# nanoporetech/pomfret

Measured on AMD Instinct MI355X. Metric: aligned reads/sec (methphase kernel), higher is better.
Workload: dtype u32/f32

## Files before the change

### include/pomfret_amd.h

```cpp
#ifndef POMFRET_AMD_H
#define POMFRET_AMD_H

#include <stddef.h>
#include <stdint.h>

#ifdef __cplusplus
extern "C" {
#endif

#define PF_ABI_VERSION 1

#define PF_OK               0
#define PF_ERR_ARG         -1
#define PF_ERR_HIP         -2
#define PF_ERR_NOMEM       -3
#define PF_ERR_UNSUPPORTED -4
#define PF_ERR_LIMIT       -5
#define PF_ERR_INTERNAL    -6

typedef struct pf_cfg {
    int32_t k;
    int32_t k_span;
    int32_t cov_for_selection;
    int32_t cov_for_runtime;
// ... 90 lines not shown
    const uint32_t *end;
    const uint64_t *cigar_off;
    const uint32_t *cigar;
    const uint64_t *seq_off;
    const uint32_t *seq_len;
    const uint8_t  *seq;
    const uint64_t *md_off;
    const char     *md;
} pf_read_aln_batch_t;


typedef struct pf_ctx pf_ctx_t;
typedef struct pf_dbatch pf_dbatch_t;

int  pf_abi_version(void);
int  pf_device_count(void);
const char *pf_strerror(int code);

int  pf_ctx_create(int device, pf_ctx_t **out);
void pf_ctx_destroy(pf_ctx_t *ctx);

int  pf_batch_upload(pf_ctx_t *ctx, const pf_cfg_t *cfg,
                     const pf_window_batch_t *batch, pf_dbatch_t **out);
void pf_batch_free(pf_dbatch_t *db);
uint32_t pf_batch_n_windows(const pf_dbatch_t *db);
uint32_t pf_batch_n_reads(const pf_dbatch_t *db);
uint64_t pf_batch_n_calls(const pf_dbatch_t *db);

int  pf_methphase_run(pf_ctx_t *ctx, pf_dbatch_t *db, pf_window_out_t *out);

int  pf_methphase_launch(pf_ctx_t *ctx, pf_dbatch_t *db);
int  pf_methphase_finish(pf_ctx_t *ctx, pf_dbatch_t *db, pf_window_out_t *out);

int  pf_batch_upload_aln(pf_ctx_t *ctx, const pf_cfg_t *cfg, const pf_load_cfg_t *lcfg,
                         const pf_aln_batch_t *aln, pf_dbatch_t **out);
int  pf_batch_read_recs(const pf_dbatch_t *db, uint32_t *rec_of_read, uint32_t n);
int64_t pf_batch_debug_calls(pf_dbatch_t *db, uint64_t *call_off, uint32_t *pos, uint8_t *cat,
                             uint32_t *first, uint32_t *last, uint64_t cap);

int  pf_batch_debug_recs(pf_dbatch_t *db, uint64_t *sizes, uint16_t *flag, uint8_t *mapq, uint32_t *pos,
                         uint32_t *l_qseq, float *de, uint8_t *hp, uint64_t *cigar_off, uint32_t *cigar,
                         uint64_t *seq_off, uint8_t *seq, uint64_t *mm_off, uint8_t *mm, uint64_t *ml_off,
                         uint8_t *ml);
int  pf_batch_load_counters(pf_dbatch_t *db, uint64_t *out, int n);

int  pf_methphase_windows(int device, const pf_cfg_t *cfg,
                          const pf_window_batch_t *batch, pf_window_out_t *out);

int  pf_last_kernel_times(pf_ctx_t *ctx, const char **names, float *ms, int *n);

int  pf_batch_stats(pf_dbatch_t *db, uint64_t *out, uint64_t n);
int  pf_batch_k3_paths(pf_dbatch_t *db, uint8_t *out, uint64_t n);
int  pf_batch_k12_paths(pf_dbatch_t *db, uint8_t *out, uint64_t n);

int  pf_batch_set_mask(pf_dbatch_t *db, const uint32_t *pos, uint64_t n, const uint32_t *win_rng);
int  pf_batch_masked_sites(pf_dbatch_t *db, uint32_t *out, uint64_t n);
int  pf_batch_k3_budget(const pf_dbatch_t *db, uint32_t *out, uint64_t n);

int  pf_batch_heavy(const pf_dbatch_t *db, uint32_t *probs, uint32_t cap);

int  pf_batch_debug_sites(pf_dbatch_t *db, uint32_t w, int dir, uint32_t *real,
                          uint32_t *starts, uint8_t *lens, uint32_t cap);
int64_t pf_batch_debug_methmers(pf_dbatch_t *db, int dir, uint32_t *mmr_n,
                                uint32_t *mmr_start, uint32_t *keys, uint64_t cap);

typedef struct pf_pileup {
    uint32_t n_windows;
    uint64_t n_sites;
    const uint64_t *win_off;
    const uint32_t *pos;
    const uint32_t *cnt;
    float ms_kernels;
} pf_pileup_t;
int  pf_batch_pileup(pf_ctx_t *ctx, pf_dbatch_t *db, const uint8_t *read_hp, uint32_t n_hp, pf_pileup_t **out);
void pf_pileup_free(pf_pileup_t *p);

typedef struct pf_dmr_cfg {
    uint32_t min_cov;
    uint32_t min_delta_pct;
    uint32_t max_gap;
    uint32_t min_sites;
} pf_dmr_cfg_t;

#define PF_DMR_OPEN_LEFT  1u
#define PF_DMR_OPEN_RIGHT 2u
typedef struct pf_dmr_run {
    uint32_t start;
    uint32_t end;
    uint32_t n_sites;
    int32_t  sign;
    uint64_t sum[4];
    uint32_t open;
    uint32_t reserved;
} pf_dmr_run_t;

typedef struct pf_dmr {
    uint64_t n_runs;
    const pf_dmr_run_t *runs;
    uint64_t n_informative;
    float ms_kernels;
    float ms_upload;
} pf_dmr_t;

int  pf_dmr_regions(pf_ctx_t *ctx, const pf_pileup_t *pile, uint32_t w0, uint32_t w1, const pf_dmr_cfg_t *cfg,
                    const uint32_t *breaks, uint32_t n_breaks, pf_dmr_t **out);
int  pf_dmr_regions_block(pf_ctx_t *ctx, const pf_pileup_t *pile, uint32_t w0, uint32_t w1, const pf_dmr_cfg_t *cfg,
// ... 490 lines not shown
```

### pomfret_amd/_lib.py

```python
from __future__ import annotations

import ctypes as C
import os
import weakref

import numpy as np

from .abi import (DMR_RUN_DTYPE, AlnBatch, AssignConfig, PfAssign, PfAssignCfg, Config, DmrConfig, KnownVars, LoadConfig, PfAlnBatch, PfCfg, PfDmr, PfDmrCfg,
                  PfKnownVars, PfLoadCfg, PfPerm, PfPileup, PfReadAlnBatch, PfTagcheck, PfWindowBatch, PfWindowOut, ReadAlnBatch,
                  WindowBatch, WindowResult)

_HERE = os.path.dirname(os.path.abspath(__file__))
LIB_PATH = os.path.join(_HERE, "libpomfret_amd.so")
_lib = None


class PomfretError(RuntimeError):
    pass


def lib():
    global _lib
    if _lib is None:
        if not os.path.exists(LIB_PATH):
# ... 547 lines not shown
    def assign(self, cfg: AssignConfig = None, read_hp=None) -> dict:
        hp_ptr, n_hp = None, 0
        if read_hp is not None:
            hp = np.zeros(np.size(read_hp) + 1, np.uint8)
            hp[:-1] = np.asarray(read_hp, np.uint8).ravel()
            hp_ptr, n_hp = hp.ctypes.data, hp.size - 1
        c = (cfg or AssignConfig()).to_c()
        p = C.POINTER(PfAssign)()
        _check(lib().pf_batch_assign(self.ctx.handle, self.handle, hp_ptr, n_hp, C.byref(c), C.byref(p)), "pf_batch_assign")
        try:
            r = p.contents
            W, R = int(r.n_windows), int(r.n_reads)

            def arr(ptr, n, dt):
                return np.ctypeslib.as_array(ptr, (n,)).copy() if n else np.zeros(0, dt)
            return dict(win_read_off=arr(r.win_read_off, W + 1, np.uint32), n_used=arr(r.n_used, R, np.uint32),
                        llr=arr(r.llr, R, np.int64), hp=arr(r.hp, R, np.uint8),
                        win_n=arr(r.win_n, 3 * W, np.uint32).reshape(W, 3), ms=float(r.ms_kernels))
        finally:
            lib().pf_assign_free(p)

    def tagcheck(self, cfg: AssignConfig = None, read_hp=None) -> dict:
        hp_ptr, n_hp = None, 0
        if read_hp is not None:
            hp = np.zeros(np.size(read_hp) + 1, np.uint8)
            hp[:-1] = np.asarray(read_hp, np.uint8).ravel()
            hp_ptr, n_hp = hp.ctypes.data, hp.size - 1
        c = (cfg or AssignConfig()).to_c()
        p = C.POINTER(PfTagcheck)()
        _check(lib().pf_batch_tagcheck(self.ctx.handle, self.handle, hp_ptr, n_hp, C.byref(c), C.byref(p)),
               "pf_batch_tagcheck")
        try:
            r = p.contents
            W, R = int(r.n_windows), int(r.n_reads)

            def arr(ptr, n, dt):
                return np.ctypeslib.as_array(ptr, (n,)).copy() if n else np.zeros(0, dt)
            return dict(win_read_off=arr(r.win_read_off, W + 1, np.uint32), n_used=arr(r.n_used, R, np.uint32),
                        llr=arr(r.llr, R, np.int64), verdict=arr(r.verdict, R, np.uint8), hp=arr(r.hp, R, np.uint8),
                        win_n=arr(r.win_n, 8 * W, np.uint32).reshape(W, 2, 4), ms=float(r.ms_kernels))
        finally:
            lib().pf_tagcheck_free(p)

    def stats(self) -> np.ndarray:
        out = np.zeros((max(self.n_windows, 1), 2, 8), np.uint64)
        _check(lib().pf_batch_stats(self.handle, out.ctypes.data, out.size), "pf_batch_stats")
        return out[:self.n_windows]

    def k12_paths(self) -> np.ndarray:
        out = np.zeros(max(self.n_windows, 1), np.uint8)
        _check(lib().pf_batch_k12_paths(self.handle, out.ctypes.data, out.size), "pf_batch_k12_paths")
        return out[:self.n_windows]

    def set_mask(self, pos, win_rng=None):
        pos = np.ascontiguousarray(np.asarray(pos, np.int64).ravel())
        if pos.size and (pos.min() < 0 or pos.max() > 0xFFFFFFFF):
            raise PomfretError("pf_batch_set_mask: positions must fit 32 bits")
        p32 = np.ascontiguousarray(pos.astype(np.uint32))
        rng = None
        if win_rng is not None:
            rng = np.ascontiguousarray(np.asarray(win_rng, np.uint32).reshape(-1))
            if rng.size != 2 * self.n_windows:
                raise PomfretError(f"pf_batch_set_mask: win_rng needs {self.n_windows} (begin, end) pairs")
        _check(lib().pf_batch_set_mask(self.handle, p32.ctypes.data if p32.size else None, p32.size,
                                       rng.ctypes.data if rng is not None and rng.size else None),
               "pf_batch_set_mask")

    def masked_sites(self) -> np.ndarray:
        out = np.zeros(max(self.n_windows, 1), np.uint32)
        _check(lib().pf_batch_masked_sites(self.handle, out.ctypes.data, out.size), "pf_batch_masked_sites")
        return out[:self.n_windows]

    def k3_paths(self) -> np.ndarray:
        out = np.zeros(max(2 * self.n_windows, 2), np.uint8)
        _check(lib().pf_batch_k3_paths(self.handle, out.ctypes.data, out.size), "pf_batch_k3_paths")
        return out[:2 * self.n_windows].reshape(-1, 2)

    def k3_budget(self) -> dict:
        out = np.zeros(4, np.uint32)
        _check(lib().pf_batch_k3_budget(self.handle, out.ctypes.data, out.size), "pf_batch_k3_budget")
        return {"lds": int(out[0]), "resident": int(out[1]), "lds_heavy": int(out[2]), "n_heavy": int(out[3])}

    def heavy_problems(self) -> np.ndarray:
        n = lib().pf_batch_heavy(self.handle, None, 0)
        out = np.zeros(max(n, 1), np.uint32)
        if n:
            lib().pf_batch_heavy(self.handle, out.ctypes.data, n)
        return out[:n]

    def debug_sites(self, w: int, direction: int, cap: int = 1 << 22):
        real = np.zeros(cap, np.uint32)
        starts = np.zeros(cap, np.uint32)
        lens = np.zeros(cap, np.uint8)
        n = lib().pf_batch_debug_sites(self.handle, w, direction, real.ctypes.data,
                                       starts.ctypes.data, lens.ctypes.data, cap)
        if n < 0:
            _check(n, "pf_batch_debug_sites")
        return real[:n], starts[:n], lens[:n]

    def debug_methmers(self, direction: int, cap: int = 1 << 26):
        n = np.zeros(max(self.n_reads, 1), np.uint32)
        st = np.zeros(max(self.n_reads, 1), np.uint32)
        keys = np.zeros(cap, np.uint32)
        tot = lib().pf_batch_debug_methmers(self.handle, direction, n.ctypes.data, st.ctypes.data,
                                            keys.ctypes.data, cap)
        if tot < 0:
# ... 33 lines not shown
```

### pomfret_amd/csrc/pf_api.hip

```cpp
#include <hip/hip_runtime.h>
#include <mutex>
#include <stdint.h>
#include <stdio.h>
#include <stdlib.h>
#include <string.h>
#include <algorithm>
#include <thread>
#include <vector>
#include "pf_device.h"
#include "pf_load.h"
#include "pf_host.h"
#include "../../include/pomfret_amd.h"

__global__ void pf_k12_sites_methmers(pf_dev_batch d);
__global__ void pf_k2_methmers(pf_dev_batch d);
__global__ void pf_k12_chunks(pf_dev_batch d);
__global__ void pf_k3_greedy(pf_dev_batch d);
__global__ void pf_k3_wave(pf_dev_batch d);
__global__ void pf_k3_fallback(pf_dev_batch d);
__global__ void pf_k3_heavy(pf_dev_batch d);
__global__ void pf_k3_kdict(pf_dev_batch d);
__global__ void pf_k0_load(pf_load_dev d);
__global__ void pf_k0_multi(pf_load_dev d);
__global__ void pf_k0_scan(pf_load_dev d);
// ... 1500 lines not shown
}

extern "C" int64_t pf_batch_debug_methmers(pf_dbatch_t *b, int dir, uint32_t *mmr_n, uint32_t *mmr_start,
                                           uint32_t *keys, uint64_t cap) {
    if (!b || dir < 0 || dir > 1) return PF_ERR_ARG;
    const int rc = run_debug(b, 2);
    if (rc) return rc;
    std::vector<uint32_t> n(2ull * b->R), s0(2ull * b->R);
    std::vector<uint64_t> off(2ull * b->R);
    if (b->R) {
        HIPCHK(hipMemcpy(n.data(), b->d.mmr_n, 8ull * b->R, hipMemcpyDeviceToHost));
        HIPCHK(hipMemcpy(s0.data(), b->d.mmr_start, 8ull * b->R, hipMemcpyDeviceToHost));
        HIPCHK(hipMemcpy(off.data(), b->d.mmr_off, 16ull * b->R, hipMemcpyDeviceToHost));
    }
    uint64_t tot = 0;
    for (uint32_t r = 0; r < b->R; r++) {
        const uint64_t g = 2ull * r + dir;
        mmr_n[r] = n[g];
        mmr_start[r] = s0[g];
        if (tot + n[g] > cap) return PF_ERR_ARG;
        if (n[g]) HIPCHK(hipMemcpy(keys + tot, b->d.keys + off[g], 4ull * n[g], hipMemcpyDeviceToHost));
        tot += n[g];
    }
    return (int64_t)tot;
}

extern "C" int pf_batch_stats(pf_dbatch_t *b, uint64_t *out, uint64_t n) {
    if (!b || !out || n < 16ull * b->W) return PF_ERR_ARG;
    HIPCHK(hipSetDevice(b->ctx->device));
    HIPCHK(hipStreamSynchronize(b->ctx->stream));
    if (b->W) HIPCHK(hipMemcpy(out, b->d.stats, 16ull * b->W * sizeof(uint64_t), hipMemcpyDeviceToHost));
    for (uint64_t i = 0; i < 2ull * b->W; i++) out[i * 8 + 2] &= (1ull << 56) - 1;
    return PF_OK;
}

extern "C" int pf_batch_k3_paths(pf_dbatch_t *b, uint8_t *out, uint64_t n) {
    if (!b || !out || n < 2ull * b->W) return PF_ERR_ARG;
    HIPCHK(hipSetDevice(b->ctx->device));
    HIPCHK(hipStreamSynchronize(b->ctx->stream));
    std::vector<uint64_t> st(16ull * b->W + 1);
    if (b->W) HIPCHK(hipMemcpy(st.data(), b->d.stats, 16ull * b->W * sizeof(uint64_t), hipMemcpyDeviceToHost));
    for (uint64_t i = 0; i < 2ull * b->W; i++) out[i] = (uint8_t)(st[i * 8 + 2] >> 56);
    return PF_OK;
}

extern "C" int pf_batch_k12_paths(pf_dbatch_t *b, uint8_t *out, uint64_t n) {
    if (!b || !out || n < b->W) return PF_ERR_ARG;
    HIPCHK(hipSetDevice(b->ctx->device));
    HIPCHK(hipStreamSynchronize(b->ctx->stream));
    if (b->W) HIPCHK(hipMemcpy(out, b->d.k12_path, b->W, hipMemcpyDeviceToHost));
    return PF_OK;
}

extern "C" int pf_batch_k3_budget(const pf_dbatch_t *b, uint32_t *out, uint64_t n) {
    if (!b || !out || n < 4) return PF_ERR_ARG;
    HIPCHK(hipSetDevice(b->ctx->device));
    out[0] = b->d.lds_bytes;
    out[1] = k3_resident(b->ctx, b->d.lds_bytes);
    out[2] = b->d.lds_heavy;
    out[3] = b->n_heavy;
    return PF_OK;
}

extern "C" int pf_batch_heavy(const pf_dbatch_t *b, uint32_t *probs, uint32_t cap) {
    if (!b) return PF_ERR_ARG;
    for (uint32_t i = 0; i < b->n_heavy && i < cap && probs; i++) probs[i] = b->h_heavy[i];
    return (int)b->n_heavy;
}

extern "C" int pf_batch_prof(pf_dbatch_t *b, uint64_t *out, uint64_t n) {
    if (!b || !out || n < 80ull * b->W) return PF_ERR_ARG;
    HIPCHK(hipSetDevice(b->ctx->device));
    HIPCHK(hipStreamSynchronize(b->ctx->stream));
    if (b->W) HIPCHK(hipMemcpy(out, b->d.prof, 80ull * b->W * sizeof(uint64_t), hipMemcpyDeviceToHost));
    return PF_OK;
}

extern "C" void pf_ctx_set_haptag_ms(pf_ctx *c, float ms, const char *name) {
    c->haptag_ms = ms; c->have_haptag = 1; c->haptag_name = name;
}

extern "C" int pf_last_kernel_times(pf_ctx_t *ctx, const char **names, float *ms, int *n) {
    if (!ctx || !n) return PF_ERR_ARG;
    const int hv = ctx->heavy_ms >= 0.0f ? 1 : 0;
    const int tot = PF_NKERN + hv + (ctx->have_haptag ? 1 : 0);
    int m = *n < tot ? *n : tot;
    for (int i = 0; i < m; i++) {
        if (i < PF_NKERN) {
            if (names) names[i] = (i == 5 && ctx->k3_block) ? "pf_k3_greedy" : k_names[i];
            if (ms) ms[i] = ctx->have_times ? ctx->last_ms[i] : -1.0f;
        } else if (i == PF_NKERN && hv) {
            if (names) names[i] = "pf_k3_heavy";
            if (ms) ms[i] = ctx->heavy_ms;
        } else {
            if (names) names[i] = ctx->haptag_name;
            if (ms) ms[i] = ctx->haptag_ms;
        }
    }
    *n = tot;
    return PF_OK;
}

extern "C" int64_t pf_batch_debug_calls(pf_dbatch_t *b, uint64_t *call_off, uint32_t *pos, uint8_t *cat,
                                        uint32_t *first, uint32_t *last, uint64_t cap) {
    if (!b || !call_off || !pos || !cat || !first || !last) return PF_ERR_ARG;
    const int rc = run_debug(b, 0);
// ... 142 lines not shown
```

### pomfret_amd/csrc/pf_kernels.hip

```cpp
#include <hip/hip_runtime.h>
#include <stdint.h>
#include "pf_device.h"

#define DEV static __device__ __forceinline__

#ifdef PF_K3_PROFILE
DEV unsigned long long k3_stamp_now() {
    unsigned long long t;
    __builtin_amdgcn_sched_barrier(0);
    asm volatile("s_memtime %0\n\ts_waitcnt lgkmcnt(0)" : "=s"(t) :: "memory");
    __builtin_amdgcn_sched_barrier(0);
    return t;
}
#define K3_STAMP(i) do { const unsigned long long t_ = k3_stamp_now(); \
    prof_acc[i] += t_ - prof_last; prof_last = t_; } while (0)
DEV unsigned long long k3_realtime() {
    unsigned long long t;
    asm volatile("s_memrealtime %0\n\ts_waitcnt lgkmcnt(0)" : "=s"(t) :: "memory");
    return t;
}
#define K3_COUNT(i, v) do { prof_acc[i] += (v); } while (0)
#define K12_STAMP(i) do { if (threadIdx.x == 0) { const unsigned long long t_ = k3_stamp_now(); \
    d.prof[64ull * d.W + (uint64_t)w * 16 + (i)] = t_ - k12_t0; k12_t0 = t_; } } while (0)
#define K2_STAMP(i) do { if (k2acc) { const unsigned long long t_ = k3_stamp_now(); \
// ... 207 lines not shown
    for (uint64_t cb = c0 + lane; cb < c1; cb += 256) {
        uint32_t pos[4], prv[4], cat[4];
#pragma unroll
        for (int u = 0; u < 4; u++) {
            const uint64_t c = cb + 64 * u;
            const bool ok = c < c1;
            pos[u] = ok ? d.call_pos[c] : 0xFFFFFFFFu;
            prv[u] = (ok && c > c0) ? d.call_pos[c - 1] : 0xFFFFFFFFu;
            cat[u] = ok ? d.call_cat[c] : 2u;
        }
#pragma unroll
        for (int u = 0; u < 4; u++) {
            const uint64_t c = cb + 64 * u;
            const uint32_t p = pos[u];
            if (c < c1 && (c == c0 || prv[u] != p) && p >= plo && p <= phi) {
                uint32_t lo = qlo, hi = qhi;
                while (lo < hi) {
                    const uint32_t mid = (lo + hi) >> 1;
                    if (sp[mid] < p) lo = mid + 1; else hi = mid;
                }
                if (lo < qhi && sp[lo] == p) chars[lo - qlo] = (uint8_t)cat[u];
            }
        }
    }
    wave_sync();
}

DEV void wave_lb2(const uint32_t *a, uint32_t n, uint32_t kA, uint32_t kB, uint32_t lane, uint32_t &lbA,
                  uint32_t &lbB) {
    const uint32_t h = lane >> 5, j = lane & 31;
    const uint32_t key = h ? kB : kA;
    uint32_t lo = 0, hi = n;
    for (;;) {
        const uint32_t len = hi - lo;
        const uint32_t step = (len + 31) >> 5;
        const uint32_t p = lo + j * step;
        const bool lt = len > 0 && p < hi && a[p] < key;
        const uint64_t bal = __ballot(lt);
        const uint32_t c = (uint32_t)__popc((uint32_t)(bal >> (32 * h)));
        if (len > 0) {
            if (c == 0) hi = lo;
            else {
                const uint32_t pn = lo + c * step;
                lo = lo + (c - 1) * step + 1;
                hi = pn < hi ? pn : hi;
            }
        }
        if (__ballot(hi > lo) == 0) break;
    }
    lbA = rdl(lo, 0);
    lbB = rdl(lo, 32);
}

struct K2SiteHash {
    const uint32_t *t;
    uint32_t mask, pmin;
};
DEV uint32_t k2_hash_slot(uint32_t rel) { return (rel * 2654435761u) >> 7; }
DEV uint32_t k2_site_of(const K2SiteHash &hs, uint32_t p) {
    const uint32_t rel = p - hs.pmin;
    if (p < hs.pmin || rel >= (1u << 19)) return PF_NONE;
    uint32_t h = k2_hash_slot(rel) & hs.mask;
    for (;;) {
        const uint32_t e = hs.t[h];
        if (e == PF_NONE) return PF_NONE;
        if ((e >> 13) == rel) return e & 8191u;
        h = (h + 1) & hs.mask;
    }
}

struct K2Read {
    uint64_t c0, c1;
    uint32_t F, L, cap, maxcall;
};

#define K2_CR 8
struct K2Calls {
    uint32_t pos[K2_CR], cat[K2_CR], site[K2_CR];
};

DEV void k2_calls_sites(K2Calls &cl, uint32_t nc, const uint32_t *sp, uint32_t S, const K2SiteHash hs,
                        bool use_hash) {
    const uint32_t sfirst = S ? sp[0] : 1u, slast = S ? sp[S - 1] : 0u;
#pragma unroll
    for (int u = 0; u < K2_CR; u++) {
        const uint32_t p = cl.pos[u];
        uint32_t si = PF_NONE;
        if (64u * u >= nc) { cl.site[u] = si; continue; }
        if (cl.cat[u] < 3u && p >= sfirst && p <= slast) {
            if (use_hash) si = k2_site_of(hs, p);
            else {
                uint32_t lo = 0, hi = S;
                while (lo < hi) {
                    const uint32_t mid = (lo + hi) >> 1;
                    if (sp[mid] < p) lo = mid + 1; else hi = mid;
                }
                si = sp[lo] == p ? lo : PF_NONE;
            }
        }
        cl.site[u] = si;
    }
}

DEV void k2_load_scalars(const pf_dev_batch &d, uint32_t r, K2Read &rd) {
    rd.c0 = d.read_call_off[r];
    rd.c1 = d.read_call_end[r];
    rd.F = d.read_first[r];
    rd.L = d.read_last[r];
    rd.cap = d.mmr_cap[r];
    rd.maxcall = 0;
}

DEV void k2_issue_calls(const pf_dev_batch &d, const K2Read &rd, uint32_t lane, uint32_t *pos, uint32_t *cat) {
    const bool fits = rd.c1 - rd.c0 <= 64ull * K2_CR && rd.cap <= d.k12_capw;
#pragma unroll
    for (int u = 0; u < K2_CR; u++) {
        const uint64_t c = rd.c0 + lane + 64u * u;
        const bool ok = fits && c < rd.c1;
        pos[u] = ok ? d.call_pos[c] : 0xFFFFFFFFu;
        cat[u] = ok ? (uint32_t)d.call_cat[c] : 3u;
    }
}

DEV void k2_finish_calls(uint64_t c0, uint64_t c1, uint32_t lane, const uint32_t *pos, const uint32_t *cat,
                         K2Calls &cl) {
    uint32_t last = 0xFFFFFFFFu;
#pragma unroll
    for (int u = 0; u < K2_CR; u++) {
        const uint64_t c = c0 + lane + 64u * u;
        uint32_t prv = (uint32_t)__builtin_amdgcn_update_dpp(0, (int)pos[u], 0x138, 0xF, 0xF, false);
        if (lane == 0) prv = last;
        last = rdl(pos[u], 63);
        cl.pos[u] = pos[u];
        cl.cat[u] = (c < c1 && (c == c0 || prv != pos[u])) ? cat[u] : 3u;
    }
}

DEV void k2_chars_reg(const K2Calls &cl, uint32_t qlo, uint32_t qhi, uint32_t lane, uint8_t *chars) {
    const uint32_t nq = qhi - qlo;
    for (uint32_t j = lane; j < nq; j += 64) chars[j] = 2;
    wave_sync();
#pragma unroll
    for (int u = 0; u < K2_CR; u++) {
        const uint32_t si = cl.site[u];
        if (si >= qlo && si < qhi) chars[si - qlo] = (uint8_t)cl.cat[u];
    }
    wave_sync();
}

template <typename IR>
DEV uint32_t k2_core(const pf_dev_batch &d, uint32_t r, uint32_t dir, uint32_t lane, uint32_t S,
                     const uint32_t *sp, const uint32_t *st, const uint8_t *lens, const uint32_t *q1,
                     uint8_t *chars, uint8_t *crank, IR *irank, uint32_t capw, const K2Read &rd,
                     const K2Calls *cl, uint64_t koff, unsigned long long *k2acc = nullptr,
                     uint32_t *kst = nullptr) {
    uint32_t staged_n = 0;
    const uint32_t g = 2 * r + dir;
    const uint64_t c0 = rd.c0, c1 = rd.c1;
    uint32_t total = 0, start_i = PF_NONE;
    if (S > 0 && c1 > c0) {
        const uint32_t F = rd.F, L = rd.L;
        const uint32_t sfirst = st[0], slast = st[S - 1];
        if (!(F > slast || L < sfirst)) {
            uint32_t lbF, lbL;
            wave_lb2(st, S, F, L, lane, lbF, lbL);
            uint32_t xl, xr;
            if (F < sfirst) xl = 0;
            else xl = st[lbF] == F ? lbF : (lbF ? lbF - 1 : 0);
            xr = L > slast ? S : lbL;
            if (xl < xr) {
                const uint32_t qlo = dir ? q1[xl] : xl;
                const uint32_t qhi = dir ? q1[xr - 1] + 1 : xr;
                const uint32_t nq = qhi - qlo;
                const uint32_t cap = rd.cap;
                if (nq > capw || xr - xl > capw) {
                    if (lane == 0) atomicOr(d.status, PF_ST_INTERNAL);
                } else {
                    K2_STAMP(0);
                    if (cl) k2_chars_reg(*cl, qlo, qhi, lane, chars);
                    else k2_chars(d, c0, c1, sp, qlo, qhi, lane, chars);
                    K2_STAMP(1);
                    uint32_t E = 0;
                    for (uint32_t i0 = xl; i0 < xr; i0 += 64) {
                        const uint32_t i = i0 + lane;
                        bool ent = false;
                        if (i < xr) ent = !(i > 1 && st[i] == st[i - 1]);
                        const uint64_t m = __ballot(ent);
                        if (ent) {
                            const uint32_t rk = E + (uint32_t)__popcll(m & lanemask_lt(lane));
                            const uint32_t q = dir ? q1[i] : i;
                            crank[rk] = chars[q - qlo];
                            irank[rk] = (IR)i;
                        }
                        E += (uint32_t)__popcll(m);
                    }
                    wave_sync();
                    K2_STAMP(2);
                    if (E > 0) {
                        const uint32_t maxcall = rd.maxcall;
                        const uint32_t usable = E - (st[irank[E - 1]] > maxcall ? 1u : 0u);
                        if (lane == 0 && E >= 2 && irank[0] == 0 && irank[1] == 1 && st[1] == st[0])
                            crank[0] = 2;
                        wave_sync();
                        uint32_t *out = d.keys + koff;
                        const uint64_t room = d.keys_cap > koff ? d.keys_cap - koff : 0;
                        for (uint32_t e0 = 0; e0 < E; e0 += 64) {
                            const uint32_t e = e0 + lane;
                            uint32_t ne = 0, fj = PF_NONE, i = 0, P = 0;
                            if (e < E) {
                                i = irank[e];
                                P = st[i];
                                for (uint32_t j = i; j < S && st[j] == P; j++) {
                                    if (e + lens[j] <= usable) {
                                        if (fj == PF_NONE) fj = j;
                                        ne++;
                                    }
                                }
                            }
                            const uint32_t incl = wave_incl_scan_dpp(ne);
                            const uint32_t tot = rdl(incl, 63);
                            if (start_i == PF_NONE && tot > 0) {
                                const uint64_t m = __ballot(ne > 0);
                                const uint32_t src = (uint32_t)__ffsll((unsigned long long)m) - 1;
                                start_i = rdl(fj, src);
                            }
                            if (ne) {
                                uint32_t pos = total + incl - ne;
                                for (uint32_t j = i; j < S && st[j] == P; j++) {
                                    const uint32_t Lj = lens[j];
                                    if (e + Lj <= usable) {
                                        uint32_t key = 0;
                                        for (uint32_t t = 0; t < Lj; t++) key = key << 2 | crank[e + t];
// ... 81 lines not shown
    const uint32_t *a = a0 + ((g & 2u) ? (a1 - a0) : 0);
    const uint32_t key = (g & 1u) ? kB : kA;
    uint32_t lo = 0, hi = n;
    for (;;) {
        const uint32_t len = hi - lo;
        const uint32_t step = (len + 15) >> 4;
        const uint32_t p = lo + j * step;
        const bool lt = len > 0 && p < hi && a[p] < key;
        const uint64_t bal = __ballot(lt);
        const uint32_t c = (uint32_t)__popc((uint32_t)(bal >> (16 * g)) & 0xFFFFu);
        if (len > 0) {
            if (c == 0) hi = lo;
            else {
                const uint32_t pn = lo + c * step;
                lo = lo + (c - 1) * step + 1;
                hi = pn < hi ? pn : hi;
            }
        }
        if (__ballot(hi > lo) == 0) break;
    }
    lbA0 = rdl(lo, 0);
    lbB0 = rdl(lo, 16);
    lbA1 = rdl(lo, 32);
    lbB1 = rdl(lo, 48);
}

DEV void k2_pack_chars(const uint8_t *cb, uint32_t n, uint32_t lane, uint32_t *pk) {
    const uint32_t *c4 = reinterpret_cast<const uint32_t *>(cb);
    for (uint32_t w = lane; 16 * w < n; w += 64) {
        uint32_t v = 0;
#pragma unroll
        for (int q = 0; q < 4; q++) {
            const uint32_t t = c4[4 * w + q] & 0x03030303u;
            v = v << 8 | (t * 0x40100401u) >> 24;
        }
        pk[w] = v;
    }
}
DEV uint64_t k2_key_window(const uint32_t *pk, uint32_t e) {
    const uint32_t w = e >> 4;
    return (uint64_t)pk[w] << 32 | pk[w + 1];
}
DEV uint32_t k2_key_of(uint64_t win, uint32_t e, uint32_t L) {
    return L ? (uint32_t)((win << (2 * (e & 15u))) >> ((64 - 2 * L) & 63u)) : 0u;
}
DEV uint32_t k2_key_bytes(const uint8_t *cb, uint32_t e, uint32_t L) {
    uint32_t key = 0;
    for (uint32_t t = 0; t < L; t++) key = key << 2 | cb[e + t];
    return key;
}

DEV bool k2_pair(const pf_dev_batch &d, uint32_t r, uint32_t lane, uint32_t S, const uint32_t *sp,
                 const uint32_t *st1, const uint32_t *q1s, const uint8_t *l0s, const uint8_t *l1s, uint8_t *wb,
                 const K2Read &rd, const K2Calls &cl, uint64_t k0, uint64_t k1, unsigned long long *k2acc,
                 uint32_t &pend_n) {
    uint8_t *chars = wb, *crank = wb + PF_K12_CAPW;
    uint16_t *irank = reinterpret_cast<uint16_t *>(wb + 2 * PF_K12_CAPW);
    uint32_t *kst = reinterpret_cast<uint32_t *>(wb + 4 * PF_K12_CAPW);
    uint32_t *pk0 = reinterpret_cast<uint32_t *>(crank), *pk1 = reinterpret_cast<uint32_t *>(chars);
    (void)pk0; (void)pk1;
    pend_n = 0;
    uint32_t xl0 = 0, xr0 = 0, xl1 = 0, xr1 = 0;
    if (S > 0 && rd.c1 > rd.c0) {
        const uint32_t F = rd.F, L = rd.L;
        const uint32_t sf0 = sp[0], sl0 = sp[S - 1], sf1 = st1[0], sl1 = st1[S - 1];
        const bool in0 = !(F > sl0 || L < sf0), in1 = !(F > sl1 || L < sf1);
        if (in0 || in1) {
            uint32_t lbF0, lbL0, lbF1, lbL1;
            wave_lb4(sp, st1, S, F, L, lane, lbF0, lbL0, lbF1, lbL1);
            if (in0) {
                xl0 = F < sf0 ? 0 : (sp[lbF0] == F ? lbF0 : (lbF0 ? lbF0 - 1 : 0));
                xr0 = L > sl0 ? S : lbL0;
            }
            if (in1) {
                xl1 = F < sf1 ? 0 : (st1[lbF1] == F ? lbF1 : (lbF1 ? lbF1 - 1 : 0));
                xr1 = L > sl1 ? S : lbL1;
            }
        }
    }
    const bool ne0 = xl0 < xr0, ne1 = xl1 < xr1;
    if (ne0 != ne1) return false;
    if (!ne0) {
        if (lane == 0) {
            d.mmr_n[2 * r] = 0; d.mmr_start[2 * r] = 0;
            d.mmr_n[2 * r + 1] = 0; d.mmr_start[2 * r + 1] = 0;
        }
        return true;
    }
    const uint32_t ql1 = q1s[xl1], qh1 = q1s[xr1 - 1] + 1;
    const uint32_t ulo = xl0 < ql1 ? xl0 : ql1, uhi = xr0 > qh1 ? xr0 : qh1;
    if (xr0 - xl0 > PF_K12_CAPW || xr1 - xl1 > PF_K12_CAPW || uhi - ulo > d.k12_capw) return false;
    K2_STAMP(0);
    k2_chars_reg(cl, ulo, uhi, lane, chars);
    const uint32_t cap = rd.cap, maxcall = rd.maxcall;
    {
        const uint32_t E = xr0 - xl0, off = xl0 - ulo;
        const uint32_t usable = E - (sp[xr0 - 1] > maxcall ? 1u : 0u);
#if PF_K12_PACK
        k2_pack_chars(chars, uhi - ulo, lane, pk0);
        wave_sync();
#endif
        K2_STAMP(1);
        const uint64_t room = d.keys_cap > k0 ? d.keys_cap - k0 : 0;
        uint32_t total = 0, start_i = PF_NONE;
        for (uint32_t e0 = 0; e0 < E; e0 += 64) {
            const uint32_t e = e0 + lane;
            bool emit = false;
            uint32_t key = 0;
            if (e < E) {
                const uint32_t Lj = l0s[xl0 + e];
#if PF_K12_PACK
                const uint64_t win = k2_key_window(pk0, off + e);
#endif
                emit = e + Lj <= usable;
#if PF_K12_PACK
                key = k2_key_of(win, off + e, Lj);
#else
                if (emit) key = k2_key_bytes(chars, off + e, Lj);
#endif
            }
            const uint64_t m = __ballot(emit);
            if (start_i == PF_NONE && m) start_i = xl0 + e0 + (uint32_t)__ffsll((unsigned long long)m) - 1;
            if (emit) {
                const uint32_t pos = total + (uint32_t)__popcll(m & lanemask_lt(lane));
                if (pos < cap && pos < room) kst[pos] = key;
            }
            total += (uint32_t)__popcll(m);
        }
        if (total > cap && lane == 0) atomicOr(d.status, PF_ST_KEYS_OVF);
        uint32_t n0 = total < cap ? total : cap;
        n0 = n0 < room ? n0 : (uint32_t)room;
        K2_STAMP(3);
        if (lane == 0) {
            d.mmr_n[2 * r] = total;
            d.mmr_start[2 * r] = total ? start_i : 0;
        }
        k2_flush(d, kst, k0, n0, lane);
        K2_STAMP(5);
    }
    {
        const uint32_t qlo = ulo;
        uint32_t E = 0;
        for (uint32_t i0 = xl1; i0 < xr1; i0 += 64) {
            const uint32_t i = i0 + lane;
            bool ent = false;
            if (i < xr1) ent = !(i > 1 && st1[i] == st1[i - 1]);
// ... 48 lines not shown
                }
                const uint32_t incl = wave_incl_scan_dpp(ne);
                const uint32_t tot = rdl(incl, 63);
                if (start_i == PF_NONE && tot > 0) {
                    const uint64_t m = __ballot(ne > 0);
                    const uint32_t src = (uint32_t)__ffsll((unsigned long long)m) - 1;
                    start_i = rdl(fj, src);
                }
                if (ne) {
                    uint32_t pos = total + incl - ne;
                    if (ne <= 8) {
                        for (uint32_t t = 0; t < ne; t++, pos++) {
                            const uint32_t Lj = (uint32_t)(lp >> (8 * t)) & 255u;
#if PF_K12_PACK
                            const uint32_t key = k2_key_of(win, e, Lj);
#else
                            const uint32_t key = k2_key_bytes(crank, e, Lj);
#endif
                            if (pos < cap && pos < room) kst[pos] = key;
                        }
                    } else {
                        for (uint32_t j = i; j < S && st1[j] == P; j++) {
                            const uint32_t Lj = l1s[j];
                            if (e + Lj <= usable) {
#if PF_K12_PACK
                                const uint32_t key = k2_key_of(win, e, Lj);
#else
                                const uint32_t key = k2_key_bytes(crank, e, Lj);
#endif
                                if (pos < cap && pos < room) kst[pos] = key;
                                pos++;
                            }
                        }
                    }
                }
                total += tot;
            }
            if (total > cap && lane == 0) atomicOr(d.status, PF_ST_KEYS_OVF);
            n1 = total < cap ? total : cap;
            n1 = n1 < room ? n1 : (uint32_t)room;
            K2_STAMP(3);
        }
        if (lane == 0) {
            d.mmr_n[2 * r + 1] = total;
            d.mmr_start[2 * r + 1] = total ? start_i : 0;
        }
        pend_n = n1;
    }
    return true;
}

DEV void k12_methmers(const pf_dev_batch &d, uint32_t r0, uint32_t i0, uint32_t i1, uint32_t wid, uint32_t NW,
                      uint32_t lane, uint32_t S, const uint32_t *sp, const uint32_t *st1, const uint32_t *q1s,
                      const uint8_t *l0s, const uint8_t *l1s, const K2SiteHash &hsd, bool use_hash, uint8_t *wb,
                      unsigned long long *k2acc, uint32_t *rctr) {
        uint8_t *chars = wb, *crank = wb + PF_K12_CAPW;
        uint16_t *irank = reinterpret_cast<uint16_t *>(wb + 2 * PF_K12_CAPW);
        uint32_t *kst = reinterpret_cast<uint32_t *>(wb + 4 * PF_K12_CAPW);
        uint32_t pend_n = 0;
        uint64_t pend_off = 0;
        auto take = [&]() -> uint32_t {
            uint32_t v = 0;
            if (lane == 0) v = atomicAdd(rctr, 1u);
            return (uint32_t)__builtin_amdgcn_readfirstlane((int)v);
        };
        K2Read rdA, rdB;
        uint32_t pA[K2_CR], tA[K2_CR], pB[K2_CR], tB[K2_CR];
        const uint32_t iw = i0 + wid;
        uint32_t iB = iw < i1 ? take() : i1;
        if (iw < i1) k2_load_scalars(d, r0 + iw, rdA);
        if (iB < i1) k2_load_scalars(d, r0 + iB, rdB);
        k2_issue_calls(d, iw < i1 ? rdA : K2Read{0, 0, 0, 0, 0, 0}, lane, pA, tA);
        for (uint32_t i = iw; i < i1;) {
            const uint32_t r = r0 + i;
            K2_STAMP(6);
            K2Read rd = rdA;
            const uint64_t nc = rd.c1 - rd.c0;
            const bool regs = rd.cap <= d.k12_capw && nc <= 64ull * K2_CR;
            K2Calls cl;
            if (regs) {
                k2_finish_calls(rd.c0, rd.c1, lane, pA, tA, cl);
                uint32_t mc = 0;
                if (nc) {
                    const uint32_t ul = (uint32_t)((nc - 1) >> 6), ll = (uint32_t)((nc - 1) & 63);
#pragma unroll
                    for (int u = 0; u < K2_CR; u++)
                        if ((uint32_t)u == ul) mc = rdl(cl.pos[u], ll);
                }
                rd.maxcall = mc;
                k2_calls_sites(cl, uni((uint32_t)nc), sp, S, hsd, use_hash);
            }
            K2_STAMP(4);
            k2_flush(d, kst, pend_off, pend_n, lane);
            pend_n = 0;
            K2Read rdC = {0, 0, 0, 0, 0, 0};
            const uint32_t iC = iB < i1 ? take() : i1;
            if (iC < i1) k2_load_scalars(d, r0 + iC, rdC);
            k2_issue_calls(d, iB < i1 ? rdB : K2Read{0, 0, 0, 0, 0, 0}, lane, pB, tB);
            K2_STAMP(8);
            if (rd.cap > d.k12_capw) {
                if (lane == 0) d.fb_list[atomicAdd(d.fb_ctr, 1u)] = r;
            } else {
                const uint64_t k0 = d.mmr_off[2ull * r], k1 = d.mmr_off[2ull * r + 1];
                if (regs) {
#if PF_K12_PAIR
                    const bool paired = k2_pair(d, r, lane, S, sp, st1, q1s, l0s, l1s, wb, rd, cl, k0, k1, k2acc, pend_n);
#else
                    const bool paired = false;
#endif
                    if (!paired) {
                        const uint32_t n0 = k2_core(d, r, 0, lane, S, sp, sp, l0s, q1s, chars, crank, irank,
                                                    PF_K12_CAPW, rd, &cl, k0, k2acc, kst);
                        k2_flush(d, kst, k0, n0, lane);
                        K2_STAMP(5);
                        pend_n = k2_core(d, r, 1, lane, S, sp, st1, l1s, q1s, chars, crank, irank, PF_K12_CAPW, rd,
                                         &cl, k1, k2acc, kst);
                    }
                    pend_off = k1;
                    K2_STAMP(5);
                } else {
                    rd.maxcall = nc ? d.call_pos[rd.c1 - 1] : 0u;
                    k2_core(d, r, 0, lane, S, sp, sp, l0s, q1s, chars, crank, irank, PF_K12_CAPW, rd, nullptr, k0);
                    k2_core(d, r, 1, lane, S, sp, st1, l1s, q1s, chars, crank, irank, PF_K12_CAPW, rd, nullptr, k1);
                }
            }
            rdA = rdB;
            rdB = rdC;
            i = iB;
            iB = iC;
#pragma unroll
            for (int u = 0; u < K2_CR; u++) { pA[u] = pB[u]; tA[u] = tB[u]; }
            K2_STAMP(7);
        }
        k2_flush(d, kst, pend_off, pend_n, lane);
}

#ifndef PF_K12_CU
#define PF_K12_CU 4
#endif
template <typename F>
DEV void k12_each_call(const pf_dev_batch &d, uint32_t r0, uint32_t R, uint32_t wid, uint32_t NW, uint32_t lane,
                       F &&f) {
    constexpr uint32_t U = PF_K12_CU;
    const uint32_t wu = (uint32_t)__builtin_amdgcn_readfirstlane((int)wid);
    for (uint32_t ib = wu; ib < R; ib += 64 * NW) {
        const uint32_t i = ib + lane * NW;
        uint32_t blo = 0, bhi = 0, n = 0;
        if (i < R) {
            const uint64_t b = d.read_call_off[r0 + i];
            blo = (uint32_t)b;
            bhi = (uint32_t)(b >> 32);
            n = (uint32_t)(d.read_call_end[r0 + i] - b);
        }
        const uint32_t cnt = min(64u, (R - ib + NW - 1) / NW);
        auto range = [&](uint32_t j, uint64_t &b, uint32_t &m) {
            const uint32_t jj = min(j, 63u);
            b = ((uint64_t)rdl(bhi, jj) << 32) | rdl(blo, jj);
            m = j < cnt ? rdl(n, jj) : 0u;
        };
        uint32_t j = 0, o = 0, cn, nn;
        uint64_t cb, nb;
        range(0, cb, cn);
        range(1, nb, nn);
        while (j < cnt) {
            uint64_t c[U];
            bool ok[U];
#pragma unroll
            for (uint32_t u = 0; u < U; u++) {
                const uint32_t rem = cn - o;
// ... 429 lines not shown
        }
        uint32_t t1, t2;
        block_excl_scan<NT>(bound, sh_scan, &t1);
        block_excl_scan<NT>(bigb, sh_scan, &t2);
        tot_keys += t1;
        tot_big += t2;
    }
    if (tid == 0) {
        const unsigned long long kb = atomicAdd(d.keys_ctr, 2ull * tot_keys);
        if (kb + 2ull * tot_keys > d.keys_cap) atomicOr(d.status, PF_ST_KEYS_OVF);
        sh_base[0] = kb;
        unsigned long long bb = 0;
        if (tot_big) {
            bb = atomicAdd(d.big_ctr, (unsigned long long)tot_big);
            if (bb + tot_big > d.big_cap) atomicOr(d.status, PF_ST_BIG_OVF);
        }
        sh_base[1] = bb;
    }
    __syncthreads();
    if (sh_base[0] + 2ull * tot_keys > d.keys_cap) {
        for (uint32_t i = tid; i < R; i += NT) {
            const uint32_t r = r0 + i;
            d.mmr_n[2 * r] = 0; d.mmr_n[2 * r + 1] = 0;
            d.mmr_start[2 * r] = 0; d.mmr_start[2 * r + 1] = 0;
            d.mmr_off[2 * r] = 0; d.mmr_off[2 * r + 1] = 0;
            d.big_off[r] = ~0ull;
        }
        if (tid == 0) d.win_S[w] = 0;
        return;
    }
    uint64_t kcarry = sh_base[0], bcarry = sh_base[1];
    for (uint32_t i0 = 0; i0 < R; i0 += NT) {
        const uint32_t i = i0 + tid;
        uint32_t bound = 0, bigb = 0;
        if (i < R) {
            bound = d.mmr_cap[r0 + i];
            if (bound > d.k2_entcap) bigb = 16 * bound;
        }
        uint32_t t1, t2;
        const uint32_t e1 = block_excl_scan<NT>(bound, sh_scan, &t1);
        const uint32_t e2 = block_excl_scan<NT>(bigb, sh_scan, &t2);
        if (i < R) {
            const uint32_t r = r0 + i;
            d.mmr_off[2 * r] = kcarry + 2ull * e1;
            d.mmr_off[2 * r + 1] = kcarry + 2ull * e1 + bound;
            d.big_off[r] = bigb ? bcarry + e2 : ~0ull;
        }
        kcarry += 2ull * t1;
        bcarry += t2;
    }

    K12_STAMP(5);
    const uint32_t arr_b = (uint32_t)((14ull * S + 15) & ~15ull);
    uint32_t HS = 1;
    while (HS < S * 4) HS <<= 1;
    const bool use_hash = staged && fast && nseg == 1 && arr_b + 4u * HS + 16u * PF_K12_WB * PF_K12_CAPW <= 4u * PF_K1_TILE;
    uint32_t *hst = reinterpret_cast<uint32_t *>(reinterpret_cast<uint8_t *>(tile) + arr_b);
    if (tid == 0) sh_misc[5] = NW;
    if (use_hash) {
        for (uint32_t j = tid; j < HS; j += NT) hst[j] = PF_NONE;
        __syncthreads();
        for (uint32_t p = tid; p < S; p += NT) {
            const uint32_t rel = sp[p] - pmin;
            uint32_t h = k2_hash_slot(rel) & (HS - 1);
            while (atomicCAS(&hst[h], PF_NONE, (rel << 13) | p) != PF_NONE) h = (h + 1) & (HS - 1);
        }
    }
    __syncthreads();
    K2SiteHash hsd;
    hsd.t = hst;
    hsd.mask = HS - 1;
    hsd.pmin = pmin;

    if (staged && R >= d.k12c_minr && S <= d.k12c_smax) {
        for (uint32_t c = tid; c * PF_K12C_READS < R; c += NT) {
            const uint32_t k = atomicAdd(d.k12c_ctr, 1u);
            d.k12c_list[2ull * k] = w;
            d.k12c_list[2ull * k + 1] = c * PF_K12C_READS;
        }
    } else if (staged) {
        uint8_t *wb = reinterpret_cast<uint8_t *>(tile) + arr_b + (use_hash ? 4u * HS : 0u) +
                      wid * (uint64_t)PF_K12_WB * PF_K12_CAPW;
#ifdef PF_K3_PROFILE
        unsigned long long k2a[10] = {0, 0, 0, 0, 0, 0, 0, 0, 0, __builtin_amdgcn_s_memtime()};
        unsigned long long *k2acc = wid == 0 ? k2a : nullptr;
#else
        unsigned long long *k2acc = nullptr;
#endif
        k12_methmers(d, r0, 0, R, wid, NW, lane, S, sp, st1, q1s, l0s, l1s, hsd, use_hash, wb, k2acc, &sh_misc[5]);
#ifdef PF_K3_PROFILE
        if (tid == 0) {
            for (int j = 0; j < 7; j++) d.prof[64ull * d.W + (uint64_t)w * 16 + 8 + j] = k2a[j];
            d.prof[64ull * d.W + (uint64_t)w * 16 + 7] = k2a[7];
            d.prof[64ull * d.W + (uint64_t)w * 16 + 15] = k2a[8];
        }
#endif
    } else {
        for (uint32_t i = tid; i < R; i += NT) d.fb_list[atomicAdd(d.fb_ctr, 1u)] = r0 + i;
    }
    __syncthreads();
    K12_STAMP(6);
}

__global__ __launch_bounds__(PF_K12C_WAVES * 64) __attribute__((amdgpu_waves_per_eu(4, 4))) void pf_k12_chunks(pf_dev_batch d) {
    extern __shared__ __attribute__((aligned(16))) uint8_t smem[];
    __shared__ uint32_t s_item, s_rctr;
    const uint32_t tid = threadIdx.x, lane = tid & 63u, wid = uni(tid >> 6);
    const uint32_t n = *d.k12c_ctr;
    for (;;) {
        if (tid == 0) s_item = atomicAdd(d.k12c_next, 1u);
        __syncthreads();
        const uint32_t it = s_item;
        if (it >= n) break;
        const uint32_t w = d.k12c_list[2ull * it], c0 = d.k12c_list[2ull * it + 1];
        if (tid == 0) s_rctr = c0 + PF_K12C_WAVES;
        const uint32_t r0 = d.win_read_off[w], R = d.win_read_off[w + 1] - r0;
        const uint32_t S = d.win_S[w];
        const uint64_t sb = d.win_site_off[w];
        uint32_t *sp = reinterpret_cast<uint32_t *>(smem), *st1 = sp + S, *q1s = sp + 2 * S;
        uint8_t *l0s = reinterpret_cast<uint8_t *>(sp + 3 * S), *l1s = l0s + S;
        for (uint32_t p = tid; p < S; p += PF_K12C_WAVES * 64) {
            sp[p] = d.site_pos[sb + p];
            st1[p] = d.st1_pos[sb + p];
            q1s[p] = d.site_q1[sb + p];
            l0s[p] = d.len0[sb + p];
            l1s[p] = d.len1[sb + p];
        }
        __syncthreads();
        const uint32_t arr_b = (uint32_t)((14ull * S + 15) & ~15ull);
        uint8_t *wb = smem + arr_b + wid * (uint64_t)PF_K12_WB * PF_K12_CAPW;
        K2SiteHash hsd;
        hsd.t = nullptr; hsd.mask = 0; hsd.pmin = 0;
        const uint32_t c1 = min(R, c0 + PF_K12C_READS);
        k12_methmers(d, r0, c0, c1, wid, PF_K12C_WAVES, lane, S, sp, st1, q1s, l0s, l1s, hsd, false, wb, nullptr,
                     &s_rctr);
        __syncthreads();
    }
}

struct K3Ctl {
    uint32_t S, R, ntot, nc, L, done, failed, inserted, winner, tag;
    int32_t i_last;
    uint32_t min_i, max_i, fail, summ, nstrict, mxlen, cmax;
    uint32_t path, need, cacheb;
    unsigned long long t_run;
    uint32_t ins_n, ins_st, ins_mo, ins_tg;
    unsigned long long scr;
    int32_t tab[4];
};

struct K3Cand {
    uint32_t read[PF_MAX_NCAND];
    uint32_t pos[PF_MAX_NCAND];
    uint32_t site0[PF_MAX_NCAND];
    uint32_t len[PF_MAX_NCAND];
    uint32_t kofs[PF_MAX_NCAND];
    unsigned long long key[PF_MAX_NCAND];
    uint8_t tag[PF_MAX_NCAND];
};

template <int NTH>
struct K3CandSlimT {
    uint32_t read[NTH];
    uint32_t pos[128];
    unsigned long long key[256];
};
using K3CandSlim = K3CandSlimT<PF_K3S_THREADS>;

DEV uint64_t align16(uint64_t x) { return (x + 15) & ~15ull; }

template <int NT, typename K, typename F>
DEV void k3_each_key(const pf_dev_batch &d, uint32_t r0, uint32_t R, uint32_t dir, K &&keep, F &&f) {
    constexpr uint32_t B = 8, NW = NT / 64;
    const uint32_t lane = threadIdx.x & 63, wid = threadIdx.x >> 6;
    for (uint32_t i0 = wid * B; i0 < R; i0 += NW * B) {
        uint32_t n[B], st[B], key[B];
        uint64_t off[B];
#pragma unroll
        for (uint32_t u = 0; u < B; u++) {
            const uint32_t i = i0 + u;
            const bool ok = i < R && keep(i);
            const uint64_t g = 2ull * (r0 + (ok ? i : 0u)) + dir;
            n[u] = ok ? d.mmr_n[g] : 0u;
            st[u] = d.mmr_start[g];
            off[u] = d.mmr_off[g];
        }
#pragma unroll
// ... 2739 lines not shown
```

Measured before the change: 57.57 million.

## Replace per-call site hash lookup with per-site binary search over staged calls

Drops the per-window site hash table and the per-call site lookups (hash or binary search over sites). Each read's calls are now packed as pos<<2|cat into LDS scratch, and each site in the query range binary-searches this sorted call array to fill the chars buffer. The calls are re-staged from global memory between the two strands because the scratch is overwritten by the flush. This frees LDS and removes the hash build, but adds a log(n) search per site, extra global reloads, and it silently drops the old duplicate-position filtering. A debug API for reading the chunk-item counter is also added.

Result: faster. 59.25 million, median of 6 (+2.9%).

```diff
diff --git a/include/pomfret_amd.h b/include/pomfret_amd.h
--- a/include/pomfret_amd.h
+++ b/include/pomfret_amd.h
@@ -166,6 +166,7 @@
 int  pf_batch_stats(pf_dbatch_t *db, uint64_t *out, uint64_t n);
 int  pf_batch_k3_paths(pf_dbatch_t *db, uint8_t *out, uint64_t n);
 int  pf_batch_k12_paths(pf_dbatch_t *db, uint8_t *out, uint64_t n);
+int  pf_batch_k12_chunk_items(pf_dbatch_t *db, uint32_t *out);
 
 int  pf_batch_set_mask(pf_dbatch_t *db, const uint32_t *pos, uint64_t n, const uint32_t *win_rng);
 int  pf_batch_masked_sites(pf_dbatch_t *db, uint32_t *out, uint64_t n);
diff --git a/pomfret_amd/_lib.py b/pomfret_amd/_lib.py
--- a/pomfret_amd/_lib.py
+++ b/pomfret_amd/_lib.py
@@ -623,6 +623,13 @@
         _check(lib().pf_batch_k12_paths(self.handle, out.ctypes.data, out.size), "pf_batch_k12_paths")
         return out[:self.n_windows]
 
+    def k12_chunk_items(self) -> int:
+        f = lib().pf_batch_k12_chunk_items
+        f.argtypes = [C.c_void_p, C.POINTER(C.c_uint32)]
+        n = C.c_uint32(0)
+        _check(f(self.handle, C.byref(n)), "pf_batch_k12_chunk_items")
+        return int(n.value)
+
     def set_mask(self, pos, win_rng=None):
         pos = np.ascontiguousarray(np.asarray(pos, np.int64).ravel())
         if pos.size and (pos.min() < 0 or pos.max() > 0xFFFFFFFF):
diff --git a/pomfret_amd/csrc/pf_api.hip b/pomfret_amd/csrc/pf_api.hip
--- a/pomfret_amd/csrc/pf_api.hip
+++ b/pomfret_amd/csrc/pf_api.hip
@@ -1576,6 +1576,14 @@
     return PF_OK;
 }
 
+extern "C" int pf_batch_k12_chunk_items(pf_dbatch_t *b, uint32_t *out) {
+    if (!b || !out) return PF_ERR_ARG;
+    HIPCHK(hipSetDevice(b->ctx->device));
+    HIPCHK(hipStreamSynchronize(b->ctx->stream));
+    HIPCHK(hipMemcpy(out, b->d.k12c_ctr, sizeof(uint32_t), hipMemcpyDeviceToHost));
+    return PF_OK;
+}
+
 extern "C" int pf_batch_k3_budget(const pf_dbatch_t *b, uint32_t *out, uint64_t n) {
     if (!b || !out || n < 4) return PF_ERR_ARG;
     HIPCHK(hipSetDevice(b->ctx->device));
diff --git a/pomfret_amd/csrc/pf_kernels.hip b/pomfret_amd/csrc/pf_kernels.hip
--- a/pomfret_amd/csrc/pf_kernels.hip
+++ b/pomfret_amd/csrc/pf_kernels.hip
@@ -283,55 +283,12 @@
     lbB = rdl(lo, 32);
 }
 
-struct K2SiteHash {
-    const uint32_t *t;
-    uint32_t mask, pmin;
-};
-DEV uint32_t k2_hash_slot(uint32_t rel) { return (rel * 2654435761u) >> 7; }
-DEV uint32_t k2_site_of(const K2SiteHash &hs, uint32_t p) {
-    const uint32_t rel = p - hs.pmin;
-    if (p < hs.pmin || rel >= (1u << 19)) return PF_NONE;
-    uint32_t h = k2_hash_slot(rel) & hs.mask;
-    for (;;) {
-        const uint32_t e = hs.t[h];
-        if (e == PF_NONE) return PF_NONE;
-        if ((e >> 13) == rel) return e & 8191u;
-        h = (h + 1) & hs.mask;
-    }
-}
-
 struct K2Read {
     uint64_t c0, c1;
     uint32_t F, L, cap, maxcall;
 };
 
 #define K2_CR 8
-struct K2Calls {
-    uint32_t pos[K2_CR], cat[K2_CR], site[K2_CR];
-};
-
-DEV void k2_calls_sites(K2Calls &cl, uint32_t nc, const uint32_t *sp, uint32_t S, const K2SiteHash hs,
-                        bool use_hash) {
-    const uint32_t sfirst = S ? sp[0] : 1u, slast = S ? sp[S - 1] : 0u;
-#pragma unroll
-    for (int u = 0; u < K2_CR; u++) {
-        const uint32_t p = cl.pos[u];
-        uint32_t si = PF_NONE;
-        if (64u * u >= nc) { cl.site[u] = si; continue; }
-        if (cl.cat[u] < 3u && p >= sfirst && p <= slast) {
-            if (use_hash) si = k2_site_of(hs, p);
-            else {
-                uint32_t lo = 0, hi = S;
-                while (lo < hi) {
-                    const uint32_t mid = (lo + hi) >> 1;
-                    if (sp[mid] < p) lo = mid + 1; else hi = mid;
-                }
-                si = sp[lo] == p ? lo : PF_NONE;
-            }
-        }
-        cl.site[u] = si;
-    }
-}
 
 DEV void k2_load_scalars(const pf_dev_batch &d, uint32_t r, K2Read &rd) {
     rd.c0 = d.read_call_off[r];
@@ -353,28 +310,30 @@
     }
 }
 
-DEV void k2_finish_calls(uint64_t c0, uint64_t c1, uint32_t lane, const uint32_t *pos, const uint32_t *cat,
-                         K2Calls &cl) {
-    uint32_t last = 0xFFFFFFFFu;
-#pragma unroll
-    for (int u = 0; u < K2_CR; u++) {
-        const uint64_t c = c0 + lane + 64u * u;
-        uint32_t prv = (uint32_t)__builtin_amdgcn_update_dpp(0, (int)pos[u], 0x138, 0xF, 0xF, false);
-        if (lane == 0) prv = last;
-        last = rdl(pos[u], 63);
-        cl.pos[u] = pos[u];
-        cl.cat[u] = (c < c1 && (c == c0 || prv != pos[u])) ? cat[u] : 3u;
-    }
-}
-
-DEV void k2_chars_reg(const K2Calls &cl, uint32_t qlo, uint32_t qhi, uint32_t lane, uint8_t *chars) {
-    const uint32_t nq = qhi - qlo;
-    for (uint32_t j = lane; j < nq; j += 64) chars[j] = 2;
+DEV void k2_stage_calls(const uint32_t *pos, const uint32_t *cat, uint32_t nc, uint32_t lane, uint32_t *cv) {
+#pragma unroll
+    for (int u = 0; u < K2_CR; u++)
+        if (64u * u + lane < nc) cv[64u * u + lane] = pos[u] << 2 | cat[u];
+}
+DEV void k2_restage_calls(const pf_dev_batch &d, uint64_t c0, uint32_t nc, uint32_t lane, uint32_t *cv) {
+    for (uint32_t c = lane; c < nc; c += 64) cv[c] = d.call_pos[c0 + c] << 2 | (uint32_t)d.call_cat[c0 + c];
+}
+
+DEV void k2_chars_site(const uint32_t *cv, uint32_t n, const uint32_t *sp, uint32_t qlo, uint32_t qhi, uint32_t lane,
+                       uint8_t *chars) {
     wave_sync();
-#pragma unroll
-    for (int u = 0; u < K2_CR; u++) {
-        const uint32_t si = cl.site[u];
-        if (si >= qlo && si < qhi) chars[si - qlo] = (uint8_t)cl.cat[u];
+    for (uint32_t q = qlo + lane; q < qhi; q += 64) {
+        const uint32_t p = sp[q], key = p << 2;
+        uint32_t base = 0;
+        for (uint32_t len = n; len > 1;) {
+            const uint32_t half = len >> 1;
+            if (cv[base + half - 1] < key) base += half;
+            len -= half;
+        }
+        uint32_t v = cv[base];
+        if (v < key) v = base + 1 < n ? cv[base + 1] : 0xFFFFFFFFu;
+        const uint32_t c = v & 3u;
+        chars[q - qlo] = (uint8_t)((v >> 2) == p && c < 2u ? c : 2u);
     }
     wave_sync();
 }
@@ -383,7 +342,7 @@
 DEV uint32_t k2_core(const pf_dev_batch &d, uint32_t r, uint32_t dir, uint32_t lane, uint32_t S,
                      const uint32_t *sp, const uint32_t *st, const uint8_t *lens, const uint32_t *q1,
                      uint8_t *chars, uint8_t *crank, IR *irank, uint32_t capw, const K2Read &rd,
-                     const K2Calls *cl, uint64_t koff, unsigned long long *k2acc = nullptr,
+                     const uint32_t *cv, uint64_t koff, unsigned long long *k2acc = nullptr,
                      uint32_t *kst = nullptr) {
     uint32_t staged_n = 0;
     const uint32_t g = 2 * r + dir;
@@ -408,7 +367,7 @@
                     if (lane == 0) atomicOr(d.status, PF_ST_INTERNAL);
                 } else {
                     K2_STAMP(0);
-                    if (cl) k2_chars_reg(*cl, qlo, qhi, lane, chars);
+                    if (cv) k2_chars_site(cv, (uint32_t)(c1 - c0), sp, qlo, qhi, lane, chars);
                     else k2_chars(d, c0, c1, sp, qlo, qhi, lane, chars);
                     K2_STAMP(1);
                     uint32_t E = 0;
@@ -596,7 +555,7 @@
 
 DEV bool k2_pair(const pf_dev_batch &d, uint32_t r, uint32_t lane, uint32_t S, const uint32_t *sp,
                  const uint32_t *st1, const uint32_t *q1s, const uint8_t *l0s, const uint8_t *l1s, uint8_t *wb,
-                 const K2Read &rd, const K2Calls &cl, uint64_t k0, uint64_t k1, unsigned long long *k2acc,
+                 const K2Read &rd, uint64_t k0, uint64_t k1, unsigned long long *k2acc,
                  uint32_t &pend_n) {
     uint8_t *chars = wb, *crank = wb + PF_K12_CAPW;
     uint16_t *irank = reinterpret_cast<uint16_t *>(wb + 2 * PF_K12_CAPW);
@@ -635,7 +594,7 @@
     const uint32_t ulo = xl0 < ql1 ? xl0 : ql1, uhi = xr0 > qh1 ? xr0 : qh1;
     if (xr0 - xl0 > PF_K12_CAPW || xr1 - xl1 > PF_K12_CAPW || uhi - ulo > d.k12_capw) return false;
     K2_STAMP(0);
-    k2_chars_reg(cl, ulo, uhi, lane, chars);
+    k2_chars_site(kst, (uint32_t)(rd.c1 - rd.c0), sp, ulo, uhi, lane, chars);
     const uint32_t cap = rd.cap, maxcall = rd.maxcall;
     {
         const uint32_t E = xr0 - xl0, off = xl0 - ulo;
@@ -790,7 +749,7 @@
 
 DEV void k12_methmers(const pf_dev_batch &d, uint32_t r0, uint32_t i0, uint32_t i1, uint32_t wid, uint32_t NW,
                       uint32_t lane, uint32_t S, const uint32_t *sp, const uint32_t *st1, const uint32_t *q1s,
-                      const uint8_t *l0s, const uint8_t *l1s, const K2SiteHash &hsd, bool use_hash, uint8_t *wb,
+                      const uint8_t *l0s, const uint8_t *l1s, uint8_t *wb,
                       unsigned long long *k2acc, uint32_t *rctr) {
         uint8_t *chars = wb, *crank = wb + PF_K12_CAPW;
         uint16_t *irank = reinterpret_cast<uint16_t *>(wb + 2 * PF_K12_CAPW);
@@ -815,22 +774,22 @@
             K2Read rd = rdA;
             const uint64_t nc = rd.c1 - rd.c0;
             const bool regs = rd.cap <= d.k12_capw && nc <= 64ull * K2_CR;
-            K2Calls cl;
             if (regs) {
-                k2_finish_calls(rd.c0, rd.c1, lane, pA, tA, cl);
                 uint32_t mc = 0;
                 if (nc) {
                     const uint32_t ul = (uint32_t)((nc - 1) >> 6), ll = (uint32_t)((nc - 1) & 63);
 #pragma unroll
                     for (int u = 0; u < K2_CR; u++)
-                        if ((uint32_t)u == ul) mc = rdl(cl.pos[u], ll);
+                        if ((uint32_t)u == ul) mc = rdl(pA[u], ll);
                 }
                 rd.maxcall = mc;
-                k2_calls_sites(cl, uni((uint32_t)nc), sp, S, hsd, use_hash);
             }
             K2_STAMP(4);
             k2_flush(d, kst, pend_off, pend_n, lane);
             pend_n = 0;
+            K2_STAMP(8);
+            if (regs) k2_stage_calls(pA, tA, uni((uint32_t)nc), lane, kst);
+            K2_STAMP(4);
             K2Read rdC = {0, 0, 0, 0, 0, 0};
             const uint32_t iC = iB < i1 ? take() : i1;
             if (iC < i1) k2_load_scalars(d, r0 + iC, rdC);
@@ -842,17 +801,18 @@
                 const uint64_t k0 = d.mmr_off[2ull * r], k1 = d.mmr_off[2ull * r + 1];
                 if (regs) {
 #if PF_K12_PAIR
-                    const bool paired = k2_pair(d, r, lane, S, sp, st1, q1s, l0s, l1s, wb, rd, cl, k0, k1, k2acc, pend_n);
+                    const bool paired = k2_pair(d, r, lane, S, sp, st1, q1s, l0s, l1s, wb, rd, k0, k1, k2acc, pend_n);
 #else
                     const bool paired = false;
 #endif
                     if (!paired) {
                         const uint32_t n0 = k2_core(d, r, 0, lane, S, sp, sp, l0s, q1s, chars, crank, irank,
-                                                    PF_K12_CAPW, rd, &cl, k0, k2acc, kst);
+                                                    PF_K12_CAPW, rd, kst, k0, k2acc, kst);
                         k2_flush(d, kst, k0, n0, lane);
+                        k2_restage_calls(d, rd.c0, (uint32_t)nc, lane, kst);
                         K2_STAMP(5);
                         pend_n = k2_core(d, r, 1, lane, S, sp, st1, l1s, q1s, chars, crank, irank, PF_K12_CAPW, rd,
-                                         &cl, k1, k2acc, kst);
+                                         kst, k1, k2acc, kst);
                     }
                     pend_off = k1;
                     K2_STAMP(5);
@@ -1388,25 +1348,8 @@
 
     K12_STAMP(5);
     const uint32_t arr_b = (uint32_t)((14ull * S + 15) & ~15ull);
-    uint32_t HS = 1;
-    while (HS < S * 4) HS <<= 1;
-    const bool use_hash = staged && fast && nseg == 1 && arr_b + 4u * HS + 16u * PF_K12_WB * PF_K12_CAPW <= 4u * PF_K1_TILE;
-    uint32_t *hst = reinterpret_cast<uint32_t *>(reinterpret_cast<uint8_t *>(tile) + arr_b);
     if (tid == 0) sh_misc[5] = NW;
-    if (use_hash) {
-        for (uint32_t j = tid; j < HS; j += NT) hst[j] = PF_NONE;
-        __syncthreads();
-        for (uint32_t p = tid; p < S; p += NT) {
-            const uint32_t rel = sp[p] - pmin;
-            uint32_t h = k2_hash_slot(rel) & (HS - 1);
-            while (atomicCAS(&hst[h], PF_NONE, (rel << 13) | p) != PF_NONE) h = (h + 1) & (HS - 1);
-        }
-    }
     __syncthreads();
-    K2SiteHash hsd;
-    hsd.t = hst;
-    hsd.mask = HS - 1;
-    hsd.pmin = pmin;
 
     if (staged && R >= d.k12c_minr && S <= d.k12c_smax) {
         for (uint32_t c = tid; c * PF_K12C_READS < R; c += NT) {
@@ -1415,15 +1358,14 @@
             d.k12c_list[2ull * k + 1] = c * PF_K12C_READS;
         }
     } else if (staged) {
-        uint8_t *wb = reinterpret_cast<uint8_t *>(tile) + arr_b + (use_hash ? 4u * HS : 0u) +
-                      wid * (uint64_t)PF_K12_WB * PF_K12_CAPW;
+        uint8_t *wb = reinterpret_cast<uint8_t *>(tile) + arr_b + wid * (uint64_t)PF_K12_WB * PF_K12_CAPW;
 #ifdef PF_K3_PROFILE
         unsigned long long k2a[10] = {0, 0, 0, 0, 0, 0, 0, 0, 0, __builtin_amdgcn_s_memtime()};
         unsigned long long *k2acc = wid == 0 ? k2a : nullptr;
 #else
         unsigned long long *k2acc = nullptr;
 #endif
-        k12_methmers(d, r0, 0, R, wid, NW, lane, S, sp, st1, q1s, l0s, l1s, hsd, use_hash, wb, k2acc, &sh_misc[5]);
+        k12_methmers(d, r0, 0, R, wid, NW, lane, S, sp, st1, q1s, l0s, l1s, wb, k2acc, &sh_misc[5]);
 #ifdef PF_K3_PROFILE
         if (tid == 0) {
             for (int j = 0; j < 7; j++) d.prof[64ull * d.W + (uint64_t)w * 16 + 8 + j] = k2a[j];
@@ -1465,10 +1407,8 @@
         __syncthreads();
         const uint32_t arr_b = (uint32_t)((14ull * S + 15) & ~15ull);
         uint8_t *wb = smem + arr_b + wid * (uint64_t)PF_K12_WB * PF_K12_CAPW;
-        K2SiteHash hsd;
-        hsd.t = nullptr; hsd.mask = 0; hsd.pmin = 0;
         const uint32_t c1 = min(R, c0 + PF_K12C_READS);
-        k12_methmers(d, r0, c0, c1, wid, PF_K12C_WAVES, lane, S, sp, st1, q1s, l0s, l1s, hsd, false, wb, nullptr,
+        k12_methmers(d, r0, c0, c1, wid, PF_K12C_WAVES, lane, S, sp, st1, q1s, l0s, l1s, wb, nullptr,
                      &s_rctr);
         __syncthreads();
     }
```
